# microsoft/Sora

Hardware: AMD Instinct MI355X
Metric: IQ Msamples/s through 802.11a 54 Mbps RX PHY (higher is better)
Workload: dtype int16 IQ / u8 path metrics

## Files before the change

### sora_amd/csrc/dev_vit16.h

```cpp
#pragma once
#include <hip/hip_runtime.h>
#include "kernels.h"
#include "dev_viterbi.h"

namespace sora {
namespace {

template <int WIN, int LOOK> struct Geom16 {
    static constexpr int kMaxWalk = (WIN + LOOK + 7) / 8 + 2;
    static constexpr int P = kMaxWalk;
    static constexpr int kPathBytes = 40;
};

template <int WIN, int LOOK> struct Lds16 {
    uint16_t ring[Geom16<WIN, LOOK>::P][4][64];
    union {
        uint32_t udump[4][64];
        uint16_t ops[4][24][2];
        uint16_t ops2[2][4][24][2];
    };
    uint32_t path[8][Geom16<WIN, LOOK>::kPathBytes / 4];
};

constexpr unsigned kW[4] = { 0u, 21u, 42u, 63u };

__device__ __forceinline__ unsigned v_of_lane(unsigned l)
{
    const unsigned b0 = l & 1u, b1 = (l >> 1) & 1u, b2 = (l >> 2) & 1u, b3 = (l >> 3) & 1u;
    const unsigned c3 = b2, c1 = b3, c0 = b0 ^ c3, c2 = b1 ^ c3;
    return c0 | (c1 << 1) | (c2 << 2) | (c3 << 3);
}
__device__ __forceinline__ unsigned lane_of_v(unsigned v)
{
    const unsigned c0 = v & 1u, c1 = (v >> 1) & 1u, c2 = (v >> 2) & 1u, c3 = (v >> 3) & 1u;
    return c0 ^ (c2 << 1) ^ (c1 << 3) ^ (c3 ? 7u : 0u);
}
__device__ __forceinline__ unsigned rev6u(unsigned x) { return __brev(x) >> 26; }

template <int CTRL> __device__ __forceinline__ unsigned dppx(unsigned v) { return (unsigned)__builtin_amdgcn_update_dpp(0, (int)v, CTRL, 0xF, 0xF, true); }

__device__ __forceinline__ unsigned partner(unsigned v, int ph)
{
    switch (ph) {
    case 0: return dppx<0x140>(v);
    case 1: return dppx<0x1B>(v);
    case 2: return dppx<0x141>(v);
    case 3: return dppx<0x4E>(v);
    case 4: return dppx<0x128>(v);
    default: return dppx<0xB1>(v);
    }
}

struct Vit16 {
    unsigned U[4];
    unsigned MX[24];
    unsigned MY[6];
    unsigned sadr[3][4];
};

template <int WHICH, int P>
__device__ __forceinline__ void acs16(Vit16& V, int t24, unsigned a, unsigned b, unsigned pos512[3])
{
    const int ph = t24 % 6, k = t24 % 8;
    const unsigned Kp = (WHICH == 0 ? 14u : 7u) * kFld + (kOne << k);
    unsigned bm;
    if (WHICH == 0)      bm = (a ^ V.MX[t24]) + (b ^ V.MY[ph]);
    else if (WHICH == 1) bm = a ^ V.MX[t24];
    else                 bm = b ^ V.MX[t24];
    const unsigned bo = Kp - bm;
    const int rx = ph == 0 ? 2 : ph == 1 ? 1 : 0;
    unsigned N[4];
#pragma unroll
    for (int i = 0; i < 4; i++) {
        const unsigned X = V.U[i], Y = partner(V.U[i ^ rx], ph);
        const bool wb = (kW[i] >> (5 - ph)) & 1u;
        N[i] = wb ? pk_min16(X + bo, Y + bm) : pk_min16(X + bm, Y + bo);
    }
#pragma unroll
    for (int i = 0; i < 4; i++) V.U[i] = N[i];
    if (k == 7) {
        const int jb = t24 / 8;
#pragma unroll
        for (int i = 0; i < 4; i++) {
            const unsigned w = bank_word(V.U[i]);
            const unsigned addr = V.sadr[jb][i] + pos512[jb];
            asm volatile("ds_write_b16 %0, %1" : : "v"(addr), "v"(w) : "memory");
            V.U[i] &= 0xFE00FE00u;
        }
    }
}

__device__ __forceinline__ unsigned row_min_u32(unsigned v)
{
    v = min(v, dppx<0xB1>(v)); v = min(v, dppx<0x4E>(v)); v = min(v, dppx<0x141>(v)); v = min(v, dppx<0x128>(v));
    return v;
}
__device__ __forceinline__ unsigned row_pkmin(unsigned v)
{
    v = pk_min16(v, dppx<0xB1>(v)); v = pk_min16(v, dppx<0x4E>(v)); v = pk_min16(v, dppx<0x141>(v)); v = pk_min16(v, dppx<0x128>(v));
    return v;
}
__device__ __forceinline__ unsigned wave_min_u32(unsigned v) { return (unsigned)__builtin_amdgcn_readfirstlane((int)dpp_min_u32_wave(v)); }
__device__ __forceinline__ unsigned wave_max_u32(unsigned v) { return ~wave_min_u32(~v); }

template <int CR, int WIN, int LOOK, int BITS>
struct Forward16 {
    static constexpr int P = Geom16<WIN, LOOK>::P, GB = Puncture<CR>::GB, GS = Puncture<CR>::GS, CW = Puncture<CR>::CW;
    static constexpr int NV = Puncture<CR>::NV;
    struct Chunk { uint32_t v[CW]; };
    struct Raw { SoftRaw r[NV]; };

    Vit16 V;
    unsigned row, half;
    uint32_t my_j;
    SoftCursor<BITS, CW> cur[NV];
    uint32_t my_base;
    const uint8_t* soft;
    uint16_t* my_ops;
    const uint4* row_ops;
    uint32_t pos;
    unsigned pos512[3];
    uint32_t tr, nsteps;
    uint32_t next_thr;
    bool all_done;

    __device__ __forceinline__ void init(Lds16<WIN, LOOK>& S, const uint8_t* __restrict__ soft_, uint32_t my_soft_off, uint32_t my_first, uint32_t my_last, unsigned start,
                                         uint32_t nsteps_)
    {
        const unsigned lane = threadIdx.x & 63, l16 = lane & 15;
        row = lane >> 4; half = lane & 1u;
        const unsigned v0 = v_of_lane(l16);
        nsteps = nsteps_;
#pragma unroll
        for (int i = 0; i < 4; i++) V.U[i] = (v0 ^ kW[i]) == 0 ? 0u : start;
        const unsigned ring_base = (unsigned)(uintptr_t)&S.ring[0][0][0];
#pragma unroll
        for (int jb = 0; jb < 3; jb++)
#pragma unroll
            for (int i = 0; i < 4; i++) V.sadr[jb][i] = ring_base + ((row * 64u + rev6u(rol6(v0 ^ kW[i], jb == 0 ? 2 : jb == 1 ? 4 : 0))) << 1);
#pragma unroll
        for (int t = 0; t < 24; t++) {
            const int ph = t % 6, k = t % 8;
            const unsigned n = rol6(v0, ph + 1);
            const bool vb = (v0 >> (5 - ph)) & 1u;
            const unsigned ma = (__popc(n & 0155) & 1) ? 7u * kFld : 0u, mb = (__popc(n & 0117) & 1) ? 7u * kFld : 0u;
            const unsigned mx = Puncture<CR>::which_of(ph) == 2 ? mb : ma;
            V.MX[t] = vb ? ((mx ^ (7u * kFld)) | (kOne << k)) : mx;
            if (t < 6) V.MY[t] = vb ? (mb ^ (7u * kFld)) : mb;
        }
        tr = 0; pos = 0;
        my_j = l16 >> 1;
#pragma unroll
        for (int v = 0; v < NV; v++) cur[v].init(my_soft_off, my_first + my_j + 8u * v, my_last);
        my_base = my_soft_off + my_first + my_j;
        soft = soft_;
        my_ops = &S.ops[row][my_j][half];
        row_ops = reinterpret_cast<const uint4*>(&S.ops[row][0][0]);
        set_row_pos();
        clear_ops(S);
    }
    __device__ __forceinline__ bool going() const { return tr < nsteps && !all_done; }

    __device__ __forceinline__ void normalize()
    {
        const unsigned m = row_pkmin(pk_min16(pk_min16(V.U[0], V.U[1]), pk_min16(V.U[2], V.U[3])));
#pragma unroll
        for (int i = 0; i < 4; i++) V.U[i] -= m;
    }
    static __device__ __forceinline__ uint32_t pos_of(uint32_t p, int jb) { const uint32_t q = p + 512u * (uint32_t)jb; return min(q, q - 512u * (uint32_t)P); }
    __device__ __forceinline__ void set_row_pos()
    {
        pos512[0] = pos; pos512[1] = pos_of(pos, 1); pos512[2] = pos_of(pos512[1], 1);
    }
    __device__ __forceinline__ void end_row() { pos = pos_of(pos512[2], 1); set_row_pos(); }
    __device__ __forceinline__ Raw fetch(uint32_t c) const
    {
        Raw R;
#pragma unroll
        for (int v = 0; v < NV; v++) R.r[v] = cur[v].fetch(soft, c);
        return R;
    }
    __device__ __forceinline__ void put(const Raw& R, uint16_t* mine) const
    {
#pragma unroll
        for (int v = 0; v < NV; v++) soft_put(mine + 16 * v, cur[v], R.r[v]);
    }
    __device__ __forceinline__ void clear_ops(Lds16<WIN, LOOK>& S) const
    {
        if constexpr (BITS == kSoftScaled) {
            static_assert(sizeof(S.ops2) == 3 * 64 * 4, "three dwords per lane");
            uint32_t* z = reinterpret_cast<uint32_t*>(&S.ops2[0][0][0][0]) + (threadIdx.x & 63);
            z[0] = 0u; z[64] = 0u; z[128] = 0u;
            lds_fence();
        }
    }
    __device__ __forceinline__ uint32_t fast_base(uint32_t c0) const { return my_base + c0 * (uint32_t)CW; }
    template <int DC> __device__ __forceinline__ Raw fetch_at(uint32_t p) const
    {
        static_assert(BITS == kSoftScaled, "one byte per value");
        Raw R;
#pragma unroll
        for (int v = 0; v < NV; v++) { R.r[v].sh = 0; R.r[v].w = soft[(size_t)p + (size_t)(DC * CW + 8 * v)]; }
        return R;
    }
    static __device__ __forceinline__ Chunk get(const uint4* table)
    {
        Chunk K;
#pragma unroll
        for (int i = 0; i < (CW + 3) / 4; i++) {
            const uint4 x = table[i];
            K.v[4 * i] = x.x; K.v[4 * i + 1] = x.y;
            if (4 * i + 2 < CW) { K.v[4 * i + 2] = x.z; K.v[4 * i + 3] = x.w; }
        }
        return K;
    }
    __device__ __forceinline__ Chunk unpack(const Raw& R) const
    {
        put(R, my_ops);
        lds_fence();
        const Chunk K = get(row_ops);
        lds_fence();
        return K;
    }
    __device__ __forceinline__ void group(const Chunk& K, int h, int i0)
    {
        const int k0 = i0 / GS * GB, t24 = 12 * h + i0;
        acs16<0, P>(V, t24, K.v[k0], K.v[k0 + 1], pos512);
        if (CR != 0) acs16<1, P>(V, t24 + 1, K.v[k0 + 2], 0, pos512);
        if (CR == 2) acs16<2, P>(V, t24 + 2, 0, K.v[k0 + 3], pos512);
        if ((t24 + GS) % 8 == 0) normalize();
    }
    __device__ __forceinline__ void fast_chunk(const Chunk& K, int h)
    {
#pragma unroll
        for (int g = 0; g < 12 / GS; g++) group(K, h, g * GS);
        tr += 12;
    }
    template <typename CHECK> __device__ __forceinline__ void slow_chunk(const Chunk& K, int h, CHECK& check)
    {
#pragma unroll
        for (int g = 0; g < 12 / GS; g++) {
            if (going()) {
                group(K, h, g * GS);
                tr += GS;
                check(12 * h + g * GS + GS - 1);
            }
        }
    }
    template <typename CHECK> __device__ __forceinline__ void chunk(const Chunk& K, int h, CHECK& check)
    {
        if (tr + 12 <= nsteps && next_thr > tr + 12) fast_chunk(K, h); else slow_chunk(K, h, check);
    }
};

template <int WIN, int LOOK, bool LANE_OB = false>
__device__ __noinline__ void trace16(unsigned lds_off, unsigned U0, unsigned U1, unsigned U2, unsigned U3, uint32_t tr_, uint32_t ob_, uint32_t pj_, uint32_t k_,
                                     uint32_t my_cnt, uint8_t* my_out)
{
    using G = Geom16<WIN, LOOK>;
    constexpr int P = G::P, K = G::kMaxWalk;
    constexpr int NR = K - 1, NF = NR / 4, NW = K / 4 + 1;
    static_assert(NR % 4 == 0 || NR % 4 == 2, "the walk's words are packed in pairs");
    static_assert(NW * 4 <= G::kPathBytes && NW >= WIN / 32 + 1, "the stream's registers hold a window and fit Lds16::path");
    typedef __attribute__((address_space(3))) Lds16<WIN, LOOK> lds_t;
    typedef __attribute__((address_space(3))) const uint16_t lds_u16;
    lds_t& S = *(lds_t*)(uintptr_t)lds_off;
    auto uni = [](uint32_t v) { return (uint32_t)__builtin_amdgcn_readfirstlane((int)v); };
    const uint32_t tr = uni(tr_), ob = LANE_OB ? ob_ : uni(ob_), pj = uni(pj_), k = uni(k_);
    const unsigned lane = threadIdx.x & 63, row = lane >> 4, l16 = lane & 15, half = lane & 1u;
    const unsigned v0 = v_of_lane(l16);
    const unsigned U[4] = { U0, U1, U2, U3 };
    const uint32_t j = (tr - 1) >> 3, nn = tr - 8u * j, m_lo = ob >> 3;
    const unsigned rowbase = (unsigned)(uintptr_t)&S.ring[0][row][0], sh = 8u * half;
    auto ring_j = [&](unsigned idx) -> unsigned { return *(lds_u16*)(uintptr_t)(rowbase + pj + (idx << 1)); };
#pragma unroll
    for (int i = 0; i < 4; i++) S.udump[i][lane] = U[i];
    lds_fence();
    unsigned key[2] = { 0xFFFFFFFFu, 0xFFFFFFFFu };
#pragma unroll
    for (int i = 0; i < 4; i++) {
        const unsigned st = rol6(v0 ^ kW[i], tr);
        unsigned lastA, lastB;
        if (k == 7) { const unsigned w = ring_j(rev6u(st)); lastA = (w >> 7) & 1u; lastB = (w >> 15) & 1u; }
        else { lastA = (U[i] >> k) & 1u; lastB = (U[i] >> (17 + k)) & 1u; }
        const unsigned mA = ((U[i] & 0xFFFFu) >> 9 << 1) | lastA, mB = (U[i] >> 25 << 1) | lastB;
        key[0] = min(key[0], (mA << 8) | (st << 2)); key[1] = min(key[1], (mB << 8) | (st << 2));
    }
    const unsigned kA = row_min_u32(key[0]), kB = row_min_u32(key[1]);
    const unsigned st = ((half ? kB : kA) >> 2) & 0x3Fu;
    const unsigned s0 = rol6(st, 6u - tr % 6u);
    const unsigned b4 = (s0 >> 4) & 1u, b5 = (s0 >> 5) & 1u;
    const unsigned ri = b4 | (b5 << 1);
    const unsigned sl = lane_of_v((s0 ^ (b4 ? 21u : 0u) ^ (b5 ? 42u : 0u)) & 15u);
    const unsigned Ust = S.udump[ri][row * 16u + sl];
    unsigned H;
    if (nn == 8) H = (ring_j(rev6u(st)) >> sh) & 0xFFu;
    else H = ((Ust >> (17u * half)) & 0xFFu) & ((1u << nn) - 1u);
    unsigned q = rev6u(((st >> nn) | rev6u(H & 0x3Fu)) & 0x3Fu);
    unsigned pr[NR / 2];
    uint32_t p = pj;
#pragma unroll
    for (int i = 1; i < K; i++) {
        uint32_t d;
        p = __builtin_sub_overflow(p, 512u, &d) ? 512u * (uint32_t)(P - 1) : d;
        unsigned base = rowbase + p;
        asm volatile("" : "+v"(base));
        const unsigned raw = *(lds_u16*)(uintptr_t)(base + (q << 1));
        q = __builtin_amdgcn_ubfe(raw, sh, 6u);
        const int s = K - 1 - i;
        if (s & 1) pr[s >> 1] = raw << 16; else pr[s >> 1] |= raw;
    }
    unsigned R[NW];
    const unsigned sel = 0x06040200u + 0x01010101u * half;
#pragma unroll
    for (int w = 0; w < NF; w++) R[w] = __builtin_amdgcn_perm(pr[2 * w + 1], pr[2 * w], sel);
    if (NR % 4 == 0) R[NF] = H;
    else R[NF] = __builtin_amdgcn_perm(H, pr[2 * NF], 0x0C040200u + 0x00000101u * half);
    const uint32_t sfirst = (uint32_t)(K - 1) - (j - m_lo);
    bool fast = !LANE_OB;
    if (!LANE_OB) {
        const bool whole = my_cnt == (uint32_t)WIN && sfirst == 1u && (((uintptr_t)my_out + m_lo) & 3u) == 0;
        fast = __ballot(!(whole || my_cnt == 0)) == 0;
    }
    if (fast) {
        if (my_cnt != 0 && l16 < 2) {
            uint32_t* o = reinterpret_cast<uint32_t*>(my_out + m_lo);
#pragma unroll
            for (int dw = 0; dw < WIN / 32; dw++) o[dw] = __builtin_amdgcn_alignbit(R[dw + 1], R[dw], 14);
        }
    } else {
        __attribute__((address_space(3))) uint32_t* pw = S.path[row * 2u + half];
        if (l16 < 2) {
#pragma unroll
            for (int w = 0; w < NW; w++) pw[w] = R[w];
        }
        lds_fence();
        __attribute__((address_space(3))) const uint8_t* pth = (__attribute__((address_space(3))) const uint8_t*)pw;
        const uint32_t nbytes = my_cnt >> 3;
        for (uint32_t z = l16 >> 1; z < nbytes; z += 8) {
            const uint32_t sb = sfirst + z;
            my_out[m_lo + z] = (uint8_t)(((unsigned)pth[sb] >> 6) | (((unsigned)pth[sb + 1] & 0x3Fu) << 2));
        }
    }
    lds_fence();
}

}
}
```

### sora_amd/csrc/dev_vitwin.h

```cpp
#pragma once
#include <hip/hip_runtime.h>
#include <type_traits>
#include "dev_vit16.h"
#include "dev_winplan.h"

namespace sora {

namespace {

struct UnitGeom {
    uint32_t soft_off, last;
    uint32_t i0;
    uint32_t nsteps;
    uint32_t ob;
    uint32_t tr_end;
    uint32_t vstep, estep;
    uint32_t wleft;
    uint32_t vec;
    uint8_t* out;
    uint32_t need;
    uint32_t idx;
    bool valid, first;
};

template <int CR, int WIN, int LOOK>
__device__ __forceinline__ UnitGeom unit_of(const VitJob& J, uint32_t idx, uint32_t uu, uint32_t m, uint32_t nun, uint32_t q, uint32_t vbase, uint8_t* __restrict__ out)
{
    constexpr uint32_t GB = Puncture<CR>::GB, GS = Puncture<CR>::GS;
    UnitGeom g;
    const bool has = uu != kWinNone;
    const uint32_t u = has ? uu : 0u;
    const uint32_t k0 = u * m, k1 = (u + 1u) * m;
    const bool last = u + 1u >= nun;
    const uint32_t b = (uint32_t)WIN * k0 / 24u * 24u;
    const uint32_t s0 = u == 0 ? 0u : b - (uint32_t)kWinWarm;
    g.valid = has; g.first = u == 0;
    g.soft_off = J.soft_off; g.last = max(J.nsoft, 1u) - 1u;
    g.i0 = s0 / GS * GB;
    g.nsteps = has ? J.nsoft / GB * GS - s0 : 0u;
    g.ob = (uint32_t)WIN * k0 - s0;
    g.tr_end = J.length * 8u + 16u + 6u - s0;
    g.vstep = (has && u != 0) ? (uint32_t)kWinWarm : kNever;
    g.estep = (has && !last) ? (uint32_t)WIN * k1 / 24u * 24u - s0 : kNever;
    g.wleft = last ? 0x10000u : m;
    g.vec = vbase + idx * q + u;
    g.out = out + J.out_off + (s0 >> 3);
    g.need = last ? J.nsoft : min(J.nsoft, (((uint32_t)WIN * k1 + (uint32_t)LOOK + 6u + GS) / GS + 1u) * GB);
    g.idx = idx;
    return g;
}

struct UnitRef { uint32_t idx, uu, m, nun; };
template <int CR, int WIN, int LOOK>
__device__ __forceinline__ UnitRef unit_ref(const VitJob& J, uint32_t n, uint32_t p, uint32_t q, bool inside, uint32_t upos, uint32_t idx)
{
    const uint32_t nev = win_events(J.length, CR, WIN, LOOK), m = win_per_unit(nev, q), nun = (nev + m - 1u) / m;
    const uint32_t uu = !inside ? kWinNone : m != 1u ? (upos < nun ? upos : kWinNone) : n == 1u ? win_unit_lone(upos, nun) : (upos < nun ? win_unit_at(upos, nun) : kWinNone);
    return UnitRef{ idx, uu, m, nun };
}
template <int CR, int WIN, int LOOK, typename JOBS>
__device__ __forceinline__ UnitGeom unit_geom(JOBS job_at, uint32_t n, uint32_t p, uint32_t q, uint32_t vbase, uint8_t* __restrict__ out)
{
    const bool inside = p < win_slots(n, q);
    const uint32_t upos = inside ? p / n : 0u, idx = inside ? p - upos * n : 0u;
    const VitJob J = job_at(idx);
    const UnitRef R = unit_ref<CR, WIN, LOOK>(J, n, p, q, inside, upos, idx);
    return unit_of<CR, WIN, LOOK>(J, idx, R.uu, R.m, R.nun, q, vbase, out);
}
template <int CR, int WIN, int LOOK, typename JOBS>
__device__ __forceinline__ UnitGeom unit_geom_direct(JOBS job_at, uint32_t idx, uint32_t u, bool exists, uint32_t q, uint32_t vbase, uint8_t* __restrict__ out)
{
    const VitJob J = job_at(idx);
    const uint32_t nev = win_events(J.length, CR, WIN, LOOK), m = win_per_unit(nev, q), nun = (nev + m - 1u) / m;
    return unit_of<CR, WIN, LOOK>(J, idx, exists && u < nun ? u : kWinNone, m, nun, q, vbase, out);
}

template <int CR, int WIN, int LOOK, int BITS, typename READY>
__device__ __forceinline__ void forward16w(Lds16<WIN, LOOK>& S, const uint8_t* __restrict__ soft, const UnitGeom& GA, const UnitGeom& GB_, uint16_t* __restrict__ vecs, READY ready)
{
    using F16 = Forward16<CR, WIN, LOOK, BITS>;
    using Raw = typename F16::Raw;
    constexpr uint32_t THR = WIN + LOOK + 6;
    const unsigned l16 = threadIdx.x & 15;
    const UnitGeom& Mine = (threadIdx.x & 1u) ? GB_ : GA;
    F16 F;
    F.init(S, soft, Mine.soft_off, Mine.i0, Mine.last, (GA.first ? 0x18u << 9 : 0u) | (GB_.first ? 0x18u << 25 : 0u), wave_max_u32(max(GA.nsteps, GB_.nsteps)));

    uint32_t my_ob = Mine.ob, my_wleft = Mine.wleft;
    const uint32_t my_tr_end = Mine.tr_end;
    bool my_done = !Mine.valid;
    uint32_t vstepA = GA.vstep, vstepB = GB_.vstep, estepA = GA.estep, estepB = GB_.estep;

    auto trace = [&](uint32_t my_cnt, int t24_last) {
        trace16<WIN, LOOK, true>((unsigned)(uintptr_t)&S, F.V.U[0], F.V.U[1], F.V.U[2], F.V.U[3], F.tr, my_ob, F16::pos_of(F.pos, t24_last / 8), (uint32_t)(t24_last % 8), my_cnt,
                                 Mine.out);
    };
    auto next_event = [&]() -> uint32_t {
        uint32_t mine = my_done ? kNever : min(my_ob + THR, my_tr_end);
        mine = min(min(mine, min(vstepA, vstepB)), min(estepA, estepB));
        return wave_min_u32(mine);
    };
    F.next_thr = next_event();
    F.all_done = wave_min_u32(my_done ? 1u : 0u) != 0u;
    auto save = [&](uint32_t vec, int which, bool hi) {
        uint16_t* d = vecs + ((size_t)vec * 2u + (uint32_t)which) * 64u + l16;
#pragma unroll
        for (int i = 0; i < 4; i++) d[16 * i] = (uint16_t)(hi ? F.V.U[i] >> 16 : F.V.U[i]);
    };
    auto check = [&](int t24_last) {
        if (F.tr >= F.next_thr) {
            if (F.tr == vstepA) { save(GA.vec, 0, false); vstepA = kNever; }
            if (F.tr == vstepB) { save(GB_.vec, 0, true); vstepB = kNever; }
            if (F.tr == estepA) { save(GA.vec, 1, false); estepA = kNever; }
            if (F.tr == estepB) { save(GB_.vec, 1, true); estepB = kNever; }
            uint32_t cnt = 0; bool partial = false;
            if (!my_done) {
                if (F.tr >= my_tr_end) { cnt = my_tr_end - my_ob - 6; my_done = true; }
                else if (F.tr >= my_ob + THR) { cnt = WIN; partial = true; }
            }
            if (wave_max_u32(cnt) != 0u) { trace(cnt, t24_last); F.clear_ops(S); }
            if (partial) { my_ob += WIN; if (--my_wleft == 0) my_done = true; }
            F.next_thr = next_event();
            F.all_done = wave_min_u32(my_done ? 1u : 0u) != 0u;
        }
    };

    uint32_t c = 0;
    if (!ready()) return;
    Raw b0 = F.fetch(0), b1 = F.fetch(1), b2, b3;
    while (F.going()) {
        const uint32_t lim = min(F.nsteps, F.next_thr - 1);
        uint32_t rows = lim > F.tr ? (lim - F.tr) / 24 : 0;
        for (; rows > 0; rows--) {
            b2 = F.fetch(c + 2);
            F.fast_chunk(F.unpack(b0), 0);
            b3 = F.fetch(c + 3);
            F.fast_chunk(F.unpack(b1), 1);
            F.end_row();
            b0 = b2; b1 = b3;
            c += 2;
        }
        if (!(F.tr < F.nsteps)) break;
        b2 = F.fetch(c + 2);
        F.chunk(F.unpack(b0), 0, check);
        if (!F.going()) break;
        b3 = F.fetch(c + 3);
        F.chunk(F.unpack(b1), 1, check);
        F.end_row();
        b0 = b2; b1 = b3;
        c += 2;
    }
}

template <int WIN, int LOOK, int BITS, typename JOBSOF, typename READY>
__device__ __forceinline__ void viterbi16w_wave(Lds16<WIN, LOOK>& S, uint32_t wave_index, JOBSOF jobs_of, READY ready, const uint32_t* __restrict__ hdr,
        uint32_t target, uint32_t vstride,
                                                const uint8_t* __restrict__ soft, uint8_t* __restrict__ out, uint16_t* __restrict__ vecs)
{
    const uint32_t n[3] = { hdr[0], hdr[1], hdr[2] };
    const uint32_t q = uni(win_units_per_frame(n[0] + n[1] + n[2], target));
    uint32_t w = uni(wave_index), list = 0;
    while (list < 3 && w >= (win_slots(n[list], q) + 7) / 8) { w -= (win_slots(n[list], q) + 7) / 8; list++; }
    if (list >= 3) return;
    const uint32_t nl = uni(n[list]);
    const auto job_at = jobs_of(list);
    const unsigned lane = threadIdx.x & 63, row = lane >> 4;
    const uint32_t pa = 8u * w + 2u * row, pb = pa + 1u, vbase = list * vstride;
    const uint32_t code_rate = uni(job_at(0).code_rate);
    auto run = [&](auto cr) {
        constexpr int CR = decltype(cr)::value;
        UnitGeom A = unit_geom<CR, WIN, LOOK>(job_at, nl, pa, q, vbase, out), B = unit_geom<CR, WIN, LOOK>(job_at, nl, pb, q, vbase, out);
        if (__ballot(A.valid || B.valid) == 0) return;
        if (!B.valid) { const bool v = false; B = A; B.valid = v; B.vstep = B.estep = kNever; B.nsteps = 0; }
        if (!A.valid) { const bool v = false; const UnitGeom T = B; A = T; A.valid = v; A.vstep = A.estep = kNever; A.nsteps = 0; }
        forward16w<CR, WIN, LOOK, BITS>(S, soft, A, B, vecs, [&]() { return ready(A, B, list); });
    };
    if (code_rate == 0) run(std::integral_constant<int, 0>{});
    else if (code_rate == 1) run(std::integral_constant<int, 1>{});
    else run(std::integral_constant<int, 2>{});
}

template <int WIN, int LOOK, int BITS>
__device__ __forceinline__ void viterbi16w_body(const VitJob* __restrict__ jobs, const uint32_t* __restrict__ hdr, uint32_t jstride, uint32_t target, uint32_t vstride,
                                                const uint8_t* __restrict__ soft, uint8_t* __restrict__ out, uint16_t* __restrict__ vecs)
{
    __shared__ Lds16<WIN, LOOK> S;
    auto jobs_of = [&](uint32_t list) { const VitJob* __restrict__ jl = jobs + (size_t)list * jstride; return [jl](uint32_t idx) { return jl[idx]; }; };
    auto ready = [](const UnitGeom&, const UnitGeom&, uint32_t) { return true; };
    viterbi16w_wave<WIN, LOOK, BITS>(S, blockIdx.x, jobs_of, ready, hdr, target, vstride, soft, out, vecs);
}

}

}
```

### sora_amd/csrc/k_vit16.hip

```cpp
#include <hip/hip_runtime.h>

#include "dev_vit16.h"

namespace sora {

namespace {

template <int CR, int WIN, int LOOK, int BITS>
__device__ __forceinline__ void forward16(Lds16<WIN, LOOK>& S, const uint8_t* __restrict__ soft, uint32_t my_soft_off, uint32_t my_nsoft,
                                          uint32_t nstepsA, uint32_t nstepsB, uint32_t my_tr_end, bool my_valid, uint8_t* my_out)
{
    using F16 = Forward16<CR, WIN, LOOK, BITS>;
    using Chunk = typename F16::Chunk;
    using Raw = typename F16::Raw;
    constexpr int GS = F16::GS;
    F16 F;
    F.init(S, soft, my_soft_off, 0, max(my_nsoft, 1u) - 1u, 0x18u * kFld, wave_max_u32(max(nstepsA, nstepsB)));

    uint32_t ob = 0;
    bool my_done = !my_valid;

    auto trace = [&](uint32_t my_cnt, int t24_last) {
        trace16<WIN, LOOK>((unsigned)(uintptr_t)&S, F.V.U[0], F.V.U[1], F.V.U[2], F.V.U[3], F.tr, ob, F16::pos_of(F.pos, t24_last / 8), (uint32_t)(t24_last % 8), my_cnt, my_out);
    };
    auto next_event = [&]() -> uint32_t {
        const uint32_t mine = my_done ? kNever : my_tr_end;
        return min(ob + (uint32_t)(WIN + LOOK + 6), wave_min_u32(mine));
    };
    F.next_thr = next_event();
    F.all_done = wave_min_u32(my_done ? 1u : 0u) != 0u;
    auto check = [&](int t24_last) {
        if (F.tr >= F.next_thr) {
            const bool partial = F.tr >= ob + (uint32_t)(WIN + LOOK + 6);
            uint32_t cnt = 0;
            if (!my_done) {
                if (F.tr >= my_tr_end) { cnt = my_tr_end - ob - 6; my_done = true; }
                else if (partial) cnt = WIN;
            }
            if (wave_max_u32(cnt) != 0u) { trace(cnt, t24_last); F.clear_ops(S); }
            if (partial) ob += WIN;
            F.next_thr = next_event();
            F.all_done = wave_min_u32(my_done ? 1u : 0u) != 0u;
        }
    };

    uint16_t* my_ops2[2] = { &S.ops2[0][F.row][F.my_j][F.half], &S.ops2[1][F.row][F.my_j][F.half] };
    const uint4* row_ops2[2] = { reinterpret_cast<const uint4*>(&S.ops2[0][F.row][0][0]), reinterpret_cast<const uint4*>(&S.ops2[1][F.row][0][0]) };
    auto stage = [&](const Raw& R, int t) { F.put(R, my_ops2[t]); };
    auto collect = [&](int t) -> Chunk { lds_fence(); return F16::get(row_ops2[t]); };
    auto fast_chunk_mid = [&](const Chunk& K, int h, Chunk& Knext, int tnext) {
#pragma unroll
        for (int g = 0; g < 12 / GS; g++) {
            if (g == (12 / GS) / 2) Knext = collect(tnext);
            F.group(K, h, g * GS);
        }
        F.tr += 12;
    };

    uint32_t c = 0;
    Raw b0 = F.fetch(0), b1 = F.fetch(1), b2, b3;
    while (F.going()) {
        const uint32_t lim = min(F.nsteps, F.next_thr - 1);
        uint32_t rows = lim > F.tr ? (lim - F.tr) / 24 : 0;
        if (rows >= 2) {
            Chunk Ka, Kb;
            b2 = F.fetch(c + 2);
            stage(b0, 0); Ka = collect(0); lds_fence();
            if constexpr (BITS == kSoftScaled) {
                uint32_t p = F.fast_base(c);
                for (; rows >= 2; rows -= 2) {
                    b3 = F.template fetch_at<3>(p); stage(b1, 1); fast_chunk_mid(Ka, 0, Kb, 1);
                    b0 = F.template fetch_at<4>(p); stage(b2, 0); fast_chunk_mid(Kb, 1, Ka, 0);
                    F.end_row();
                    b1 = F.template fetch_at<5>(p); stage(b3, 1); fast_chunk_mid(Ka, 0, Kb, 1);
                    b2 = F.template fetch_at<6>(p); stage(b0, 0); fast_chunk_mid(Kb, 1, Ka, 0);
                    F.end_row();
                    c += 4; p += 4u * (uint32_t)F16::CW;
                }
            } else {
                for (; rows >= 2; rows -= 2) {
                    b3 = F.fetch(c + 3); stage(b1, 1); fast_chunk_mid(Ka, 0, Kb, 1);
                    b0 = F.fetch(c + 4); stage(b2, 0); fast_chunk_mid(Kb, 1, Ka, 0);
                    F.end_row();
                    b1 = F.fetch(c + 5); stage(b3, 1); fast_chunk_mid(Ka, 0, Kb, 1);
                    b2 = F.fetch(c + 6); stage(b0, 0); fast_chunk_mid(Kb, 1, Ka, 0);
                    F.end_row();
                    c += 4;
                }
            }
            lds_fence();
        }
        if (!(F.tr < F.nsteps)) break;
        b2 = F.fetch(c + 2);
        if (rows) F.fast_chunk(F.unpack(b0), 0); else F.chunk(F.unpack(b0), 0, check);
        if (!F.going()) break;
        b3 = F.fetch(c + 3);
        if (rows) F.fast_chunk(F.unpack(b1), 1); else F.chunk(F.unpack(b1), 1, check);
        F.end_row();
        b0 = b2; b1 = b3;
        c += 2;
    }
}

template <int WIN, int LOOK, int BITS>
__device__ __forceinline__ void viterbi16_body(const VitJob* __restrict__ jobs, const uint32_t* __restrict__ njobs3, uint32_t njobs_single, uint32_t stride,
                                               const uint8_t* __restrict__ soft, uint8_t* __restrict__ out)
{
    __shared__ Lds16<WIN, LOOK> S;
    uint32_t n[3] = { njobs_single, 0, 0 };
    if (njobs3) { n[0] = njobs3[0]; n[1] = njobs3[1]; n[2] = njobs3[2]; }
    uint32_t w = uni(blockIdx.x), list = 0;
    while (list < 3 && w >= (n[list] + 7) / 8) { w -= (n[list] + 7) / 8; list++; }
    if (list >= 3) return;
    const uint32_t njobs = uni(n[list]);
    jobs += (size_t)list * stride;
    const unsigned lane = threadIdx.x & 63, row = lane >> 4, half = lane & 1u;
    const uint32_t fa = 8u * w + 2u * row, fb = fa + 1u;
    const bool hasA = fa < njobs, hasB = fb < njobs;
    const VitJob& GA = jobs[hasA ? fa : 8u * w];
    const VitJob& GBj = jobs[hasB ? fb : (hasA ? fa : 8u * w)];
    const uint32_t code_rate = uni(jobs[8u * w].code_rate);
    const uint32_t gsd = code_rate == 0 ? 2u : code_rate == 2 ? 4u : 3u, gss = code_rate == 0 ? 1u : code_rate == 2 ? 3u : 2u;
    const uint32_t nstepsA = hasA ? GA.nsoft / gsd * gss : 0u, nstepsB = hasB ? GBj.nsoft / gsd * gss : 0u;
    const VitJob& Mine = half ? GBj : GA;
    const bool my_valid = half ? hasB : hasA;
    const uint32_t my_tr_end = Mine.length * 8u + 16u + 6u;
    uint8_t* my_out = out + Mine.out_off;
    if (code_rate == 0)      forward16<0, WIN, LOOK, BITS>(S, soft, Mine.soft_off, Mine.nsoft, nstepsA, nstepsB, my_tr_end, my_valid, my_out);
    else if (code_rate == 1) forward16<1, WIN, LOOK, BITS>(S, soft, Mine.soft_off, Mine.nsoft, nstepsA, nstepsB, my_tr_end, my_valid, my_out);
    else                     forward16<2, WIN, LOOK, BITS>(S, soft, Mine.soft_off, Mine.nsoft, nstepsA, nstepsB, my_tr_end, my_valid, my_out);
}

}

__global__ void __launch_bounds__(64) k_viterbi16(const VitJob* __restrict__ jobs, const uint32_t* __restrict__ njobs3, uint32_t njobs_single, uint32_t stride,
        const uint8_t* __restrict__ soft, uint8_t* __restrict__ out)
{ viterbi16_body<256, 24, kSoftScaled>(jobs, njobs3, njobs_single, stride, soft, out); }
__global__ void __launch_bounds__(64) k_viterbi16_p3(const VitJob* __restrict__ jobs, const uint32_t* __restrict__ njobs3, uint32_t njobs_single, uint32_t stride,
        const uint8_t* __restrict__ soft, uint8_t* __restrict__ out)
{ viterbi16_body<256, 24, 3>(jobs, njobs3, njobs_single, stride, soft, out); }
__global__ void __launch_bounds__(64) k_viterbi16_11n(const VitJob* __restrict__ jobs, const uint32_t* __restrict__ njobs3, uint32_t njobs_single,
        uint32_t stride, const uint8_t* __restrict__ soft, uint8_t* __restrict__ out)
{ viterbi16_body<192, 36, 8>(jobs, njobs3, njobs_single, stride, soft, out); }

}
```

Measured before the change: 55800.

## Rework Viterbi traceback start to avoid LDS state dump and ring wrap arithmetic

The traceback no longer dumps the four survivor registers to LDS to look up the winning state's history. It now builds packed min-keys with byte permutes that carry both the state and its history bits, so the best state and its history come straight out of the row minimum. The ring walk precomputes a wrap mask and picks between two bases per step with immediate offsets, replacing the per-step subtract-with-wrap. The clear_ops call after each trace is dropped because the udump union member that overlapped ops is no longer written. This is dense bit-level logic and carries a correctness risk.

```diff
diff --git a/sora_amd/csrc/dev_vit16.h b/sora_amd/csrc/dev_vit16.h
--- a/sora_amd/csrc/dev_vit16.h
+++ b/sora_amd/csrc/dev_vit16.h
@@ -15,7 +15,7 @@
 template <int WIN, int LOOK> struct Lds16 {
     uint16_t ring[Geom16<WIN, LOOK>::P][4][64];
     union {
-        uint32_t udump[4][64];
+        uint32_t spare[4][64];
         uint16_t ops[4][24][2];
         uint16_t ops2[2][4][24][2];
     };
@@ -254,72 +254,72 @@
 };
 
 template <int WIN, int LOOK, bool LANE_OB = false>
-__device__ __noinline__ void trace16(unsigned lds_off, unsigned U0, unsigned U1, unsigned U2, unsigned U3, uint32_t tr_, uint32_t ob_, uint32_t pj_, uint32_t k_,
-                                     uint32_t my_cnt, uint8_t* my_out)
+__device__ __noinline__ void trace16(unsigned lds_off, unsigned U0, unsigned U1, unsigned U2, unsigned U3, uint32_t tr_, uint32_t ob_, uint32_t pj_, uint8_t* my_out, uint32_t my_cnt)
 {
     using G = Geom16<WIN, LOOK>;
     constexpr int P = G::P, K = G::kMaxWalk;
     constexpr int NR = K - 1, NF = NR / 4, NW = K / 4 + 1;
     static_assert(NR % 4 == 0 || NR % 4 == 2, "the walk's words are packed in pairs");
     static_assert(NW * 4 <= G::kPathBytes && NW >= WIN / 32 + 1, "the stream's registers hold a window and fit Lds16::path");
+    static_assert(512 * (K - 1) < 65536, "the walk's offsets fit ds_read_u16's immediate");
     typedef __attribute__((address_space(3))) Lds16<WIN, LOOK> lds_t;
     typedef __attribute__((address_space(3))) const uint16_t lds_u16;
     lds_t& S = *(lds_t*)(uintptr_t)lds_off;
     auto uni = [](uint32_t v) { return (uint32_t)__builtin_amdgcn_readfirstlane((int)v); };
-    const uint32_t tr = uni(tr_), ob = LANE_OB ? ob_ : uni(ob_), pj = uni(pj_), k = uni(k_);
-    const unsigned lane = threadIdx.x & 63, row = lane >> 4, l16 = lane & 15, half = lane & 1u;
-    const unsigned v0 = v_of_lane(l16);
-    const unsigned U[4] = { U0, U1, U2, U3 };
-    const uint32_t j = (tr - 1) >> 3, nn = tr - 8u * j, m_lo = ob >> 3;
-    const unsigned rowbase = (unsigned)(uintptr_t)&S.ring[0][row][0], sh = 8u * half;
-    auto ring_j = [&](unsigned idx) -> unsigned { return *(lds_u16*)(uintptr_t)(rowbase + pj + (idx << 1)); };
-#pragma unroll
-    for (int i = 0; i < 4; i++) S.udump[i][lane] = U[i];
-    lds_fence();
-    unsigned key[2] = { 0xFFFFFFFFu, 0xFFFFFFFFu };
+    const uint32_t tr = uni(tr_), ob = LANE_OB ? ob_ : uni(ob_), pj = uni(pj_);
+    const uint32_t k = (tr - 1u) & 7u, nn = k + 1u, j = (tr - 1u) >> 3, m_lo = ob >> 3;
+    const unsigned lane = threadIdx.x & 63, row = lane >> 4, l16 = lane & 15;
+    const bool half = lane & 1u;
+    const unsigned rowbase = (unsigned)(uintptr_t)&S.ring[0][row][0], sh = half ? 8u : 0u;
+    const unsigned r = rol6(v_of_lane(l16), tr);
+    const uint32_t a = (tr & 1u) ? 42u : 21u;
+    const uint32_t cst[4] = { 0u, a, a ^ 63u, 63u };
+    unsigned U[4] = { U0, U1, U2, U3 }, st4[4] = { r, r ^ cst[1], r ^ cst[2], r ^ cst[3] };
+    asm volatile("" : "+v"(st4[1]), "+v"(st4[2]), "+v"(st4[3]));
+    if (k == 7) {
+#pragma unroll
+        for (int i = 0; i < 4; i++) {
+            const unsigned w = *(lds_u16*)(uintptr_t)(rowbase + pj + (rev6u(st4[i]) << 1));
+            U[i] |= (w | (w << 9)) & 0x01FE00FFu;
+        }
+    }
+    const uint32_t last = 0x10000u << k, mskA = 0xFE00FFFFu | last, mskB = 0x7F00FFFFu | last;
+    unsigned key[2][4];
 #pragma unroll
     for (int i = 0; i < 4; i++) {
-        const unsigned st = rol6(v0 ^ kW[i], tr);
-        unsigned lastA, lastB;
-        if (k == 7) { const unsigned w = ring_j(rev6u(st)); lastA = (w >> 7) & 1u; lastB = (w >> 15) & 1u; }
-        else { lastA = (U[i] >> k) & 1u; lastB = (U[i] >> (17 + k)) & 1u; }
-        const unsigned mA = ((U[i] & 0xFFFFu) >> 9 << 1) | lastA, mB = (U[i] >> 25 << 1) | lastB;
-        key[0] = min(key[0], (mA << 8) | (st << 2)); key[1] = min(key[1], (mB << 8) | (st << 2));
-    }
-    const unsigned kA = row_min_u32(key[0]), kB = row_min_u32(key[1]);
-    const unsigned st = ((half ? kB : kA) >> 2) & 0x3Fu;
-    const unsigned s0 = rol6(st, 6u - tr % 6u);
-    const unsigned b4 = (s0 >> 4) & 1u, b5 = (s0 >> 5) & 1u;
-    const unsigned ri = b4 | (b5 << 1);
-    const unsigned sl = lane_of_v((s0 ^ (b4 ? 21u : 0u) ^ (b5 ? 42u : 0u)) & 15u);
-    const unsigned Ust = S.udump[ri][row * 16u + sl];
-    unsigned H;
-    if (nn == 8) H = (ring_j(rev6u(st)) >> sh) & 0xFFu;
-    else H = ((Ust >> (17u * half)) & 0xFFu) & ((1u << nn) - 1u);
-    unsigned q = rev6u(((st >> nn) | rev6u(H & 0x3Fu)) & 0x3Fu);
+        key[0][i] = __builtin_amdgcn_perm(U[i], st4[i], 0x05040004u) & mskA;
+        key[1][i] = __builtin_amdgcn_perm(U[i] >> 1, st4[i], 0x07060006u) & mskB;
+    }
+    const unsigned kA = row_min_u32(min(min(key[0][0], key[0][1]), min(key[0][2], key[0][3])));
+    const unsigned kB = row_min_u32(min(min(key[1][0], key[1][1]), min(key[1][2], key[1][3])));
+    const unsigned kk = half ? kB : kA;
+    const unsigned H = kk & ((1u << nn) - 1u);
+    unsigned q = ((__brev(kk) >> (18u - nn)) | H) & 0x3Fu;
+    const unsigned baseN = rowbase + pj - 512u * (uint32_t)(K - 1), baseW = baseN + 512u * (uint32_t)P;
+    static_assert(K <= 63, "one bit per block of the walk");
+    const uint64_t wrapped = ~0ull << ((pj >> 9) + 1u);
     unsigned pr[NR / 2];
-    uint32_t p = pj;
 #pragma unroll
     for (int i = 1; i < K; i++) {
-        uint32_t d;
-        p = __builtin_sub_overflow(p, 512u, &d) ? 512u * (uint32_t)(P - 1) : d;
-        unsigned base = rowbase + p;
-        asm volatile("" : "+v"(base));
-        const unsigned raw = *(lds_u16*)(uintptr_t)(base + (q << 1));
+        uint64_t every;
+        unsigned base;
+        asm("s_bfe_i64 %0, %1, %2" : "=s"(every) : "s"(wrapped), "n"(0x10000 | i) : "scc");
+        asm("v_cndmask_b32_e64 %0, %1, %2, %3" : "=v"(base) : "v"(baseN), "v"(baseW), "s"(every));
+        const unsigned raw = *(lds_u16*)(uintptr_t)(base + (q << 1) + 512u * (uint32_t)(K - 1 - i));
         q = __builtin_amdgcn_ubfe(raw, sh, 6u);
         const int s = K - 1 - i;
         if (s & 1) pr[s >> 1] = raw << 16; else pr[s >> 1] |= raw;
     }
     unsigned R[NW];
-    const unsigned sel = 0x06040200u + 0x01010101u * half;
+    const unsigned sel = half ? 0x07050301u : 0x06040200u;
 #pragma unroll
     for (int w = 0; w < NF; w++) R[w] = __builtin_amdgcn_perm(pr[2 * w + 1], pr[2 * w], sel);
     if (NR % 4 == 0) R[NF] = H;
-    else R[NF] = __builtin_amdgcn_perm(H, pr[2 * NF], 0x0C040200u + 0x00000101u * half);
+    else R[NF] = __builtin_amdgcn_perm(H, pr[2 * NF], half ? 0x0C040301u : 0x0C040200u);
     const uint32_t sfirst = (uint32_t)(K - 1) - (j - m_lo);
     bool fast = !LANE_OB;
     if (!LANE_OB) {
-        const bool whole = my_cnt == (uint32_t)WIN && sfirst == 1u && (((uintptr_t)my_out + m_lo) & 3u) == 0;
+        const bool whole = my_cnt == (uint32_t)WIN && sfirst == 1u && (((uint32_t)(uintptr_t)my_out + m_lo) & 3u) == 0;
         fast = __ballot(!(whole || my_cnt == 0)) == 0;
     }
     if (fast) {
@@ -329,7 +329,9 @@
             for (int dw = 0; dw < WIN / 32; dw++) o[dw] = __builtin_amdgcn_alignbit(R[dw + 1], R[dw], 14);
         }
     } else {
-        __attribute__((address_space(3))) uint32_t* pw = S.path[row * 2u + half];
+        const unsigned fr = ((lane >> 3) & 6u) | (half ? 1u : 0u);
+        static_assert(G::kPathBytes == 40, "path rows are addressed by two shifts");
+        __attribute__((address_space(3))) uint32_t* pw = (__attribute__((address_space(3))) uint32_t*)(uintptr_t)((unsigned)(uintptr_t)&S.path[0][0] + (fr << 5) + (fr << 3));
         if (l16 < 2) {
 #pragma unroll
             for (int w = 0; w < NW; w++) pw[w] = R[w];
diff --git a/sora_amd/csrc/dev_vitwin.h b/sora_amd/csrc/dev_vitwin.h
--- a/sora_amd/csrc/dev_vitwin.h
+++ b/sora_amd/csrc/dev_vitwin.h
@@ -92,8 +92,7 @@
     uint32_t vstepA = GA.vstep, vstepB = GB_.vstep, estepA = GA.estep, estepB = GB_.estep;
 
     auto trace = [&](uint32_t my_cnt, int t24_last) {
-        trace16<WIN, LOOK, true>((unsigned)(uintptr_t)&S, F.V.U[0], F.V.U[1], F.V.U[2], F.V.U[3], F.tr, my_ob, F16::pos_of(F.pos, t24_last / 8), (uint32_t)(t24_last % 8), my_cnt,
-                                 Mine.out);
+        trace16<WIN, LOOK, true>((unsigned)(uintptr_t)&S, F.V.U[0], F.V.U[1], F.V.U[2], F.V.U[3], F.tr, my_ob, F16::pos_of(F.pos, t24_last / 8), Mine.out, my_cnt);
     };
     auto next_event = [&]() -> uint32_t {
         uint32_t mine = my_done ? kNever : min(my_ob + THR, my_tr_end);
@@ -118,7 +117,7 @@
                 if (F.tr >= my_tr_end) { cnt = my_tr_end - my_ob - 6; my_done = true; }
                 else if (F.tr >= my_ob + THR) { cnt = WIN; partial = true; }
             }
-            if (wave_max_u32(cnt) != 0u) { trace(cnt, t24_last); F.clear_ops(S); }
+            if (wave_max_u32(cnt) != 0u) trace(cnt, t24_last);
             if (partial) { my_ob += WIN; if (--my_wleft == 0) my_done = true; }
             F.next_thr = next_event();
             F.all_done = wave_min_u32(my_done ? 1u : 0u) != 0u;
diff --git a/sora_amd/csrc/k_vit16.hip b/sora_amd/csrc/k_vit16.hip
--- a/sora_amd/csrc/k_vit16.hip
+++ b/sora_amd/csrc/k_vit16.hip
@@ -21,7 +21,7 @@
     bool my_done = !my_valid;
 
     auto trace = [&](uint32_t my_cnt, int t24_last) {
-        trace16<WIN, LOOK>((unsigned)(uintptr_t)&S, F.V.U[0], F.V.U[1], F.V.U[2], F.V.U[3], F.tr, ob, F16::pos_of(F.pos, t24_last / 8), (uint32_t)(t24_last % 8), my_cnt, my_out);
+        trace16<WIN, LOOK>((unsigned)(uintptr_t)&S, F.V.U[0], F.V.U[1], F.V.U[2], F.V.U[3], F.tr, ob, F16::pos_of(F.pos, t24_last / 8), my_out, my_cnt);
     };
     auto next_event = [&]() -> uint32_t {
         const uint32_t mine = my_done ? kNever : my_tr_end;
@@ -37,7 +37,7 @@
                 if (F.tr >= my_tr_end) { cnt = my_tr_end - ob - 6; my_done = true; }
                 else if (partial) cnt = WIN;
             }
-            if (wave_max_u32(cnt) != 0u) { trace(cnt, t24_last); F.clear_ops(S); }
+            if (wave_max_u32(cnt) != 0u) trace(cnt, t24_last);
             if (partial) ob += WIN;
             F.next_thr = next_event();
             F.all_done = wave_min_u32(my_done ? 1u : 0u) != 0u;
```

Result: no change. 56550, median of 6 (+1.4%).
